# PrinceVictor/LWSNet

Measured on AMD Instinct MI355X. Metric: stereo pairs/sec @256x512 maxdisp=192 (stage-4), higher is better.
Workload: dtype f32; 1 GPU; BASELINE config 2: batch=1/GPU, 256x512 synthetic pair, maxdisplist=[24,5,5], all 4 stages; pairs_per_gpu=1, streams=1, parallelism=single GPU, weights=seeded synthetic (seed 7, calibrated BN), GPU_MAX_HW_QUEUES=4

## Files before the change

lwsnet_amd/csrc/lws_api.hip:

```cpp
#include <stdarg.h>
#include <stdio.h>
#include <string.h>

#include <algorithm>

#include "lws_common.h"

namespace lws {

static thread_local char g_err[512] = "";
thread_local hipEvent_t tl_stop_event = nullptr;

void set_error(const char *fmt, ...)
{
    va_list ap;
    va_start(ap, fmt);
    vsnprintf(g_err, sizeof(g_err), fmt, ap);
    va_end(ap);
}

static constexpr int kClockWgs = 64;

int check_device(const lws_ctx *h, const char *what)
{
    int cur = -1;
    if (hipGetDevice(&cur) != hipSuccess) {
        (void)hipGetLastError();
        cur = -1;
    }
    if (cur != h->device) {
        set_error("%s: the handle belongs to HIP device %d but the calling thread's current device is %d "
                  "(hipSetDevice(%d) first; -1 = no device)", what, h->device, cur, h->device);
        return LWS_ERR_INVALID;
    }
    return LWS_OK;
}

void apply_options(lws_ctx *h)
{
    for (int i = 0; i < 3; ++i) {
        h->stage[i].mid16_split = (h->opt.split_bf16 & 1) != 0;
        h->stage[i].mid8_split = (h->opt.split_bf16 & 2) != 0;
        h->stage[i].mid8_balance = h->mid8_balance;
        h->stage[i].cu_count = h->cu_count;
    }
    h->net2d.r2_first.form = (h->opt.split_bf16 & 4) ? 1 : 0;
}

}

using namespace lws;

extern "C" {

int lws_abi_version(void) { return LWS_ABI_VERSION; }

const char *lws_last_error(void) { return g_err; }

int lws_device_count(void)
{
    int n = 0;
    if (hipGetDeviceCount(&n) != hipSuccess) return 0;
    return n;
}

int lws_create(const lws_config *cfg, lws_handle *out)
{
    LWS_CHECK_ARG(cfg != nullptr && out != nullptr, "lws_create: null argument");
    LWS_CHECK_ARG(cfg->layers_3d >= 1 && cfg->layers_3d <= 16, "layers_3d must be in 1..16 (got %d)", cfg->layers_3d);
    LWS_CHECK_ARG(cfg->maxdisplist[0] >= 1 && cfg->maxdisplist[0] <= 64, "maxdisplist[0] must be in 1..64 (got %d)",
                  cfg->maxdisplist[0]);
    for (int i = 1; i < 3; ++i)
        LWS_CHECK_ARG(cfg->maxdisplist[i] >= 1 && 2 * cfg->maxdisplist[i] - 1 <= 64,
                      "maxdisplist[%d] must be in 1..32 (got %d)", i, cfg->maxdisplist[i]);
    for (int i = 0; i < 3; ++i) {
        const int c3 = cfg->channels_3d * cfg->growth_rate[i];
        LWS_CHECK_ARG(c3 == 8 || c3 == 16 || c3 == 32,
                      "stage %d: channels_3d*growth_rate = %d is not supported by the gfx950 kernels (8, 16, 32)", i, c3);
    }
    LWS_CHECK_ARG(cfg->feature_fp16 == 0 || cfg->feature_fp16 == 1, "feature_fp16 must be 0 or 1 (got %d)", cfg->feature_fp16);
    LWS_CHECK_ARG(cfg->interp_align_mode == 0 || cfg->interp_align_mode == 1, "interp_align_mode must be 0 or 1 (got %d)",
                  cfg->interp_align_mode);
    lws_ctx *h = new (std::nothrow) lws_ctx();
    if (!h) {
        set_error("out of host memory");
        return LWS_ERR_NOMEM;
    }
    h->cfg = *cfg;
    h->spec = build_spec(*cfg);
    for (int i = 0; i < 3; ++i) h->stage[i].c3 = cfg->channels_3d * cfg->growth_rate[i];
    if (hipGetDevice(&h->device) != hipSuccess) h->device = -1;
    (void)hipGetLastError();
    *out = h;
    return LWS_OK;
}

static int *option_slot(lws_ctx *h, const char *name)
{
    struct { const char *name; int *slot; } tab[] = {{"fuse_first", &h->opt.fuse_first},
                                                     {"defer_upsample", &h->opt.defer_upsample},
                                                     {"side_streams", &h->opt.side_streams},
                                                     {"split_bf16", &h->opt.split_bf16},
                                                     {"ref_chunk_mb", &h->opt.ref_chunk_mb},
                                                     {"ref_pipe", &h->opt.ref_pipe},
                                                     {"warp_form", &h->opt.warp_form},
                                                     {"fuse_last1", &h->opt.fuse_last1},
                                                     {"fork2_after", &h->opt.fork2_after},
                                                     {"fuse_ref_last", &h->opt.fuse_ref_last},
                                                     {"host_joins", &h->opt.host_joins},
                                                     {"host_join_budget_us", &h->opt.host_join_budget_us},
                                                     {"device", &h->device}};
    for (auto &e : tab)
        if (strcmp(e.name, name) == 0) return e.slot;
    return nullptr;
}

int lws_set_option(lws_handle h, const char *name, int value)
{
    LWS_CHECK_ARG(h && name, "lws_set_option: null argument");
    int *slot = option_slot(h, name);
    LWS_CHECK_ARG(slot != nullptr, "lws_set_option: unknown option '%s'", name);
    if (strcmp(name, "split_bf16") == 0)
        LWS_CHECK_ARG(value >= 0 && value <= 7, "lws_set_option: split_bf16 is a bit mask in 0..7 (got %d)", value);
    else if (strcmp(name, "fuse_first") == 0)
        LWS_CHECK_ARG(value >= 0 && value <= 3, "lws_set_option: fuse_first is a bit mask in 0..3 (got %d)", value);
    else if (strcmp(name, "ref_pipe") == 0 || strcmp(name, "fuse_ref_last") == 0 || strcmp(name, "host_joins") == 0)
        LWS_CHECK_ARG(value >= -1 && value <= 1, "lws_set_option: %s is out of range (got %d)", name, value);
    else if (strcmp(name, "host_join_budget_us") == 0)
        LWS_CHECK_ARG(value >= 0 && value <= 1000000, "lws_set_option: host_join_budget_us must be in 0..1000000 (got %d)", value);
    else if (strcmp(name, "ref_chunk_mb") == 0)
        LWS_CHECK_ARG(value >= 0 && value <= 4096, "lws_set_option: ref_chunk_mb must be in 0..4096 (got %d)", value);
    else if (strcmp(name, "device") == 0) {
        LWS_CHECK_ARG(value >= 0, "lws_set_option: device must be >= 0 (got %d)", value);
        LWS_CHECK_ARG(h->params == nullptr && h->ws == nullptr && h->side == nullptr,
                      "lws_set_option: the device of a handle can only be changed before lws_finalize / lws_reserve "
                      "have allocated on device %d", h->device);
    }
    else if (strcmp(name, "fork2_after") == 0)
        LWS_CHECK_ARG(value >= -1 && value <= 16, "lws_set_option: fork2_after must be in -1..16 (got %d)", value);
    else
        LWS_CHECK_ARG(value == 0 || value == 1, "lws_set_option: %s must be 0 or 1 (got %d)", name, value);
    *slot = value;
    apply_options(h);
    return LWS_OK;
}

int lws_get_option(lws_handle h, const char *name, int *value)
{
    LWS_CHECK_ARG(h && name && value, "lws_get_option: null argument");
    int *slot = option_slot(h, name);
    LWS_CHECK_ARG(slot != nullptr, "lws_get_option: unknown option '%s'", name);
    *value = *slot;
    return LWS_OK;
}

int lws_profile_enable(lws_handle h, int class_mask)
{
    LWS_CHECK_ARG(h, "lws_profile_enable: null handle");
    prof_clear(h);
    h->prof_mask = h->prof_mask_cfg = (unsigned)class_mask;
    h->prof_every = 1;
    h->prof_calls = 0;
    return LWS_OK;
}

int lws_profile_sample(lws_handle h, int every_n)
{
    LWS_CHECK_ARG(h && every_n >= 1, "lws_profile_sample: every_n must be >= 1");
    h->prof_every = every_n;
    h->prof_calls = 0;
    return LWS_OK;
}

int lws_profile_read(lws_handle h, double *total_ms, int64_t *launches)
{
    LWS_CHECK_ARG(h && total_ms && launches, "lws_profile_read: null argument");
    LWS_CHECK_DEVICE(h, "lws_profile_read");
    for (int i = 0; i < LWS_KC_COUNT; ++i) {
        total_ms[i] = 0.0;
        launches[i] = 0;
    }
    for (lws_prof_rec &r : h->prof) {
        LWS_HIP(hipEventSynchronize(r.t1));
        float ms = 0.f;
        LWS_HIP(hipEventElapsedTime(&ms, r.t0, r.t1));
        total_ms[r.kc] += ms;
        launches[r.kc] += 1;
    }
    return LWS_OK;
}

int lws_profile_read_class(lws_handle h, int kernel_class, float *ms_out, int capacity, int *count)
{
    LWS_CHECK_ARG(h && count && (ms_out || capacity == 0) && capacity >= 0, "lws_profile_read_class: bad argument");
    LWS_CHECK_ARG(kernel_class >= 0 && kernel_class < LWS_KC_COUNT, "lws_profile_read_class: unknown kernel class %d", kernel_class);
    LWS_CHECK_DEVICE(h, "lws_profile_read_class");
    int n = 0;
    for (lws_prof_rec &r : h->prof) {
        if (r.kc != kernel_class) continue;
        if (n < capacity) {
            LWS_HIP(hipEventSynchronize(r.t1));
            float ms = 0.f;
            LWS_HIP(hipEventElapsedTime(&ms, r.t0, r.t1));
            ms_out[n] = ms;
        }
        ++n;
    }
    *count = n;
    return LWS_OK;
// ... 134 lines not shown
```

lwsnet_amd/csrc/lws_common.h:

```cpp
#pragma once
#include <hip/hip_runtime.h>
#include <hip/hip_ext.h>
#include <stdint.h>

#include <atomic>
#include <map>
#include <string>
#include <type_traits>
#include <vector>

#include "lwsnet_hip.h"

namespace lws {

void set_error(const char *fmt, ...) __attribute__((format(printf, 1, 2)));

#define LWS_CHECK_ARG(cond, ...)                 \
    do {                                         \
        if (!(cond)) {                           \
            ::lws::set_error(__VA_ARGS__);       \
            return LWS_ERR_INVALID;              \
        }                                        \
    } while (0)

// ... 114 lines not shown
    }
#define LWS_STAMPK(k, i)                 \
    do {                                 \
        if ((k) == LWS_STAMPS) stamp_(i); \
    } while (0)
#else
#define LWS_DEFINE_STAMPS(tu)
#define LWS_STAMPK(k, i) do {} while (0)
#endif

struct Conv3dLayer {
    int cin = 0, cout = 0;
    float *w = nullptr;
    float *bn_s = nullptr;
    float *bn_t = nullptr;
    float *w_mfma = nullptr;
};

struct Stage3d {
    int c3 = 0;
    bool mid8_split = false;
    bool mid16_split = false;
    int mid8_balance = 1;
    int cu_count = 0;
    unsigned long long *clk = nullptr;
    std::vector<Conv3dLayer> layers;
};

struct Conv2dLayer {
    int cin = 0, cout = 0, stride = 1, pad = 1, dil = 1;
    bool transposed = false, relu = false;
    float *w = nullptr, *bn_s = nullptr, *bn_t = nullptr;
    float *w_pair = nullptr;
    float *w_mfma = nullptr;
    int pair_groups = 0;
};

struct RefDws {
    int dil = 1;
    float *bn_s = nullptr, *bn_t = nullptr;
    float *dw = nullptr;
    float *pw = nullptr;
};

struct RefConv64 {
    float *bn_s = nullptr, *bn_t = nullptr;
    float *w = nullptr;
    float *wx = nullptr;
    int form = 0;
};

struct Net2d {
    Conv2dLayer fe[12];
    float *r1_first[2] = {nullptr, nullptr};
    float *r1_first_mfma[2] = {nullptr, nullptr};
    RefDws r1[2][4];
    RefConv64 r2_first;
    RefDws r2[4];
    float *r2_last = nullptr;
};

}

struct lws_join_stat {
    int64_t host = 0, queued = 0, wait_ns = 0, max_ns = 0;
};

struct lws_prof_rec {
    int kc;
    hipEvent_t t0, t1;
};

struct lws_ctx {
    lws_config cfg;
    struct {
        int fuse_first = 3;
        int defer_upsample = 1;
        int side_streams = 1;
        int split_bf16 = 0;
        int ref_pipe = -1;
        int warp_form = 1;
        int fuse_last1 = 1;
        int fork2_after = -1;
        int fuse_ref_last = -1;
        int ref_chunk_mb = 72;
        int host_joins = -1;
        int host_join_budget_us = 900;
    } opt;
    lws_join_stat join_stat[3];
    unsigned prof_mask = 0;
    unsigned prof_mask_cfg = 0;
    int prof_every = 1;
    unsigned prof_calls = 0;
    std::vector<lws_prof_rec> prof;
    std::vector<hipEvent_t> evt_pool;
    int device = 0;
    int cu_count = 0;
    bool finalized = false;
    std::map<std::string, std::vector<float>> host;
    std::map<std::string, std::vector<int64_t>> shapes;
    std::map<std::string, std::vector<int64_t>> spec;
    float *params = nullptr;
    bool owns_params = true;
    size_t params_bytes = 0;
    lws::Stage3d stage[3];
    lws::Net2d net2d;
    bool have_2d = false;
    float *ws = nullptr;
    size_t ws_bytes = 0;
    int mid8_balance = 1;
    hipStream_t side = nullptr;
    hipEvent_t ev_fork = nullptr, ev_join = nullptr;
    hipEvent_t ev_feat[3] = {nullptr, nullptr, nullptr};
    hipEvent_t ev_fork2 = nullptr;
    unsigned long long *clk_buf = nullptr;
};

namespace lws {

struct StageMap {
    float *mem = nullptr;
    bool written = false;
    const float *low = nullptr;
    int h = 0, w = 0;
    StageMap *prev = nullptr;
};
int check_stage_map(const StageMap &m, bool nested, const char *who);

int check_device(const lws_ctx *h, const char *what);
#define LWS_CHECK_DEVICE(h, what)                     \
    do {                                              \
        int rc_dev_ = ::lws::check_device((h), what); \
        if (rc_dev_) return rc_dev_;                  \
    } while (0)
void apply_options(lws_ctx *h);
void prof_clear(lws_ctx *h);
std::map<std::string, std::vector<int64_t>> build_spec(const lws_config &cfg);

int launch_volume_l1_shift(const float *L, const float *R, float *cost, int B, int C, int h, int w, int D,
                           hipStream_t st, bool q16 = false);
int launch_volume_l1_warp(const float *L, const float *R, StageMap &prev, float *cost, float *wflow_out,
                          int B, int C, int h, int w, int H, int W, int m, hipStream_t st, bool q16 = false,
                          int form = 1,
                          float ioff = 0.5f);
int launch_softargmin(const float *cost, float *low, int B, int D, int h, int w, float start, hipStream_t st);
int launch_upsample_add(const float *low, const float *prev, float *out, int B, int h, int w, int H, int W,
                        hipStream_t st, float ioff = 0.5f);
int launch_softargmin_upsample(const float *cost, const float *prev, float *out, float *low_out, int B, int D, int h,
                               int w, int H, int W, float start, hipStream_t st, float ioff = 0.5f);
int launch_softargmin_conf(const float *cost, float *disp_low, float *peak_low, float *sigma_low, float *conf, float *sigma, int B,
                           int D, int h, int w, int H, int W, float start, hipStream_t st, float ioff = 0.5f);

bool shift_first_can_fuse(const Stage3d &s, int C);
int launch_shift_first(const Stage3d &s, const float *L, const float *R, float *cost, float *act_out, int B, int C, int D,
                       int h, int w, hipStream_t st, bool q16);
int launch_conv3d_first(const Stage3d &s, const float *cost, float *act_out, int B, int D, int h, int w,
                        hipStream_t st);
int launch_conv3d_mid(const Stage3d &s, int layer, const float *act_in, float *act_out, int B, int D, int h,
                      int w, hipStream_t st, hipEvent_t e0 = nullptr, hipEvent_t e1 = nullptr);
int launch_conv3d_last(const Stage3d &s, const float *act_in, const float *cost_skip, float *cost_out, int B,
                       int D, int h, int w, hipStream_t st);

int launch_conv2d_nchw(const Conv2dLayer &l, const float *in, const float *res, float *out, int N, int H, int W,
                       hipStream_t st, const float *in2 = nullptr, int n1 = 0);
int conv2d_pair_groups(int layer);
void pack_pair_mfma(const float *w, int cin, float *out);
// ... 30 lines not shown
```

lwsnet_amd/csrc/lws_feature2d.hip:

```cpp
#include "lws_common.h"
#include "lws_device_math.h"

namespace lws {

LWS_DEFINE_STAMPS(feature2d)

template <int CIN, int COUT, bool TRANSPOSED>
__global__ __launch_bounds__(256) void k_conv2d_nchw(const float *__restrict__ in, const float *__restrict__ in2, int n1,
                                                     const float *__restrict__ wgt,
                                                     const float *__restrict__ bn_s, const float *__restrict__ bn_t,
                                                     const float *__restrict__ res, float *__restrict__ out, int H,
                                                     int W, int Ho, int Wo, int stride, int pad, int dil, int relu,
                                                     int RH, int RW, int RWp)
{
    constexpr int CPT = COUT / 4;
    extern __shared__ float sIn[];
    const int b = blockIdx.z;
    const int tid = threadIdx.x, tx = tid & 7, ty = (tid >> 3) & 7;
    const int wave_id = __builtin_amdgcn_readfirstlane(tid >> 6);
    const int co0 = wave_id * CPT;
    const int ox0 = blockIdx.x * 8, oy0 = blockIdx.y * 8;
    const int ry0 = TRANSPOSED ? ((oy0 - 1) >> 1) : oy0 * stride - pad;
    const int rx0 = TRANSPOSED ? ((ox0 - 1) >> 1) : ox0 * stride - pad;
    const int plane = H * W, oplane = Ho * Wo;
    const float *inb = b < n1 ? in + (int64_t)b * CIN * plane : in2 + (int64_t)(b - n1) * CIN * plane;
    LWS_STAMPK(7, 0);
    const int rsz = RH * RW;
#pragma unroll
    for (int k = 0; k < 2; ++k) {
        const int r = tid + 256 * k;
        if (r < rsz) {
            const int ry = r / RW, rx = r - ry * RW;
            const int gy = ry0 + ry, gx = rx0 + rx;
            const bool ok = gy >= 0 && gy < H && gx >= 0 && gx < W;
            const float *src = inb + (ok ? gy * W + gx : 0);
            float v[CIN];
#pragma unroll
            for (int ci = 0; ci < CIN; ++ci) v[ci] = src[ci * plane];
            float *dst = sIn + ry * RWp + rx;
#pragma unroll
            for (int ci = 0; ci < CIN; ++ci) dst[ci * RH * RWp] = ok ? v[ci] : 0.0f;
        }
    }
    __syncthreads();
    LWS_STAMPK(7, 1);
    const int ox = ox0 + tx, oy = oy0 + ty;
    if (ox >= Wo || oy >= Ho) return;
    float acc[CPT];
#pragma unroll
    for (int c = 0; c < CPT; ++c) acc[c] = 0.0f;
    const int cstride = RH * RWp;
#pragma unroll 3
    for (int tap = 0; tap < 9; ++tap) {
        const int kh = tap / 3, kw = tap - kh * 3;
        int ly, lx;
        bool ok = true;
        if (TRANSPOSED) {
            const int t_y = oy + 1 - kh, t_x = ox + 1 - kw;
            ok = t_y >= 0 && !(t_y & 1) && (t_y >> 1) < H && t_x >= 0 && !(t_x & 1) && (t_x >> 1) < W;
            ly = (t_y >> 1) - ry0;
            lx = (t_x >> 1) - rx0;
        } else {
            ly = ty * stride + kh * dil;
            lx = tx * stride + kw * dil;
        }
        const float *p = sIn + (ok ? ly * RWp + lx : 0);
        const float *w = wgt + (tap * 4 + wave_id) * CIN * CPT;
        float v[CIN];
#pragma unroll
        for (int ci = 0; ci < CIN; ++ci) v[ci] = ok ? p[ci * cstride] : 0.0f;
#pragma unroll
        for (int ci = 0; ci < CIN; ++ci)
#pragma unroll
            for (int c = 0; c < CPT; ++c) acc[c] = fmaf(v[ci], w[ci * CPT + c], acc[c]);
    }
    LWS_STAMPK(7, 2);
    const int64_t o = ((int64_t)b * COUT + co0) * oplane + oy * Wo + ox;
#pragma unroll
    for (int c = 0; c < CPT; ++c) {
        float v = acc[c];
        if (bn_s != nullptr) v = fmaf(v, bn_s[co0 + c], bn_t[co0 + c]);
        if (res != nullptr) v = v + res[o + (int64_t)c * oplane];
        if (relu) v = fmaxf(v, 0.0f);
        out[o + (int64_t)c * oplane] = v;
    }
    LWS_STAMPK(7, 3);
}

template <int CIN, int COUT, bool TR>
static int conv2d_launch(const Conv2dLayer &l, const float *in, const float *in2, int n1, const float *res, float *out,
                         int N, int H, int W, int Ho, int Wo, hipStream_t st)
{
    const int RH = TR ? 6 : 7 * l.stride + 2 * l.dil + 1, RW = RH;
    const int RWp = RW | 1;
    const size_t lds = (size_t)CIN * RH * RWp * sizeof(float);
    dim3 grid(cdiv(Wo, 8), cdiv(Ho, 8), N), block(256);
    hipLaunchKernelGGL((k_conv2d_nchw<CIN, COUT, TR>), grid, block, lds, st, in, in2, n1, l.w, l.bn_s, l.bn_t, res, out, H,
                       W, Ho, Wo, l.stride, l.pad, l.dil, l.relu ? 1 : 0, RH, RW, RWp);
    LWS_LAUNCH_CHECK();
    return LWS_OK;
}

int launch_conv2d_nchw(const Conv2dLayer &l, const float *in, const float *res, float *out, int N, int H, int W,
                       hipStream_t st, const float *in2, int n1)
{
    if (in2 == nullptr) {
        in2 = in;
        n1 = N;
    }
    int Ho, Wo;
    if (l.transposed) {
        Ho = 2 * H;
        Wo = 2 * W;
    } else {
        Ho = (H + 2 * l.pad - 2 * l.dil - 1) / l.stride + 1;
        Wo = (W + 2 * l.pad - 2 * l.dil - 1) / l.stride + 1;
    }
#define LWS_C2D(CI, CO, TR)                                   \
    if (l.cin == CI && l.cout == CO && l.transposed == TR)    \
        return conv2d_launch<CI, CO, TR>(l, in, in2, n1, res, out, N, H, W, Ho, Wo, st);
    LWS_C2D(3, 4, false) LWS_C2D(4, 8, false) LWS_C2D(8, 4, false) LWS_C2D(8, 16, false) LWS_C2D(16, 16, false)
    LWS_C2D(16, 16, true) LWS_C2D(16, 8, true) LWS_C2D(8, 8, false)
#undef LWS_C2D
    set_error("conv2d_nchw: unsupported layer cin=%d cout=%d", l.cin, l.cout);
    return LWS_ERR_INVALID;
}

template <int CIN, int CM, int COUT, int SA, int DA, int DB, int NW>
struct PairCfg {
    static constexpr int NT = 64 * NW;
    static constexpr int MR = 8 + 2 * DB, MRp = MR | 1;
    static constexpr int RH = (MR - 1) * SA + 2 * DA + 1;
    static constexpr int HALF = (RH + 1) / 2, RWp = (SA == 2 ? 2 * HALF : RH) | 1;
    __host__ __device__ static constexpr int col(int rx) { return SA == 2 ? (rx & 1) * HALF + (rx >> 1) : rx; }
    static constexpr int WGA_ = (MR * MR + 63) / 64;
    static constexpr int WGA = WGA_ <= 1 ? 1 : WGA_ <= 2 ? 2 : WGA_ <= 4 ? 4 : WGA_ <= 8 ? 8 : 16;
    static constexpr int GA = NW / WGA, CPA = CM / GA, CPB = COUT / NW;
    static constexpr int ITEMS = CIN * RH * RH, SITER = (ITEMS + NT - 1) / NT;
    static constexpr int LDS_FLOATS = CIN * RH * RWp + CM * MR * MRp;
    static_assert(WGA <= NW && NW % WGA == 0 && CM % GA == 0 && COUT % NW == 0 && CPA >= 1 && CPB >= 1, "bad pair geometry");
    static_assert(WGA * 64 >= MR * MR, "phase 2 must be one pass");
};

template <int CIN, int CM, int COUT, int SA, int DA, int DB, int NW>
__global__ __launch_bounds__(64 * NW) void k_conv2d_pair(const float *__restrict__ in, const float *__restrict__ in2, int n1,
                                                         const float *__restrict__ wA, const float *__restrict__ sA_,
                                                         const float *__restrict__ tA_, int reluA,
                                                         const float *__restrict__ wB, const float *__restrict__ sB_,
                                                         const float *__restrict__ tB_, const float *__restrict__ res,
                                                         int reluB, float *__restrict__ out, int H, int W, int HA, int WA)
{
    using Cfg = PairCfg<CIN, CM, COUT, SA, DA, DB, NW>;
    constexpr int NT = Cfg::NT, MR = Cfg::MR, MRp = Cfg::MRp, RH = Cfg::RH, RWp = Cfg::RWp, WGA = Cfg::WGA, GA = Cfg::GA,
                  CPA = Cfg::CPA, CPB = Cfg::CPB, SITER = Cfg::SITER, RSZ = RH * RH;
    extern __shared__ float smem[];
    float *sIn = smem;
    float *sMid = smem + CIN * RH * RWp;
    const int b = blockIdx.z;
    const int tid = threadIdx.x, lane = tid & 63, wave = __builtin_amdgcn_readfirstlane(tid >> 6);
    const int ox0 = blockIdx.x * 8, oy0 = blockIdx.y * 8;
    const int my0 = oy0 - DB, mx0 = ox0 - DB;
    const int iy0 = my0 * SA - DA, ix0 = mx0 * SA - DA;
    const int plane = H * W;
    const float *inb = b < n1 ? in + (int64_t)b * CIN * plane : in2 + (int64_t)(b - n1) * CIN * plane;
    [[maybe_unused]] constexpr int STAMP_ID = 13 + (CIN == 3 ? 0 : CM == 4 ? 1 : CIN == 8 ? 2 : 3);
    LWS_STAMPK(STAMP_ID, 0);
    {
        float v[SITER];
        bool okv[SITER];
#pragma unroll
        for (int i = 0; i < SITER; ++i) {
            const int it = tid + i * NT;
            const int ci = it / RSZ, r = it - ci * RSZ;
            const int ry = r / RH, rx = r - ry * RH;
            const int gy = iy0 + ry, gx = ix0 + rx;
            okv[i] = it < Cfg::ITEMS && gy >= 0 && gy < H && gx >= 0 && gx < W;
            v[i] = inb[okv[i] ? ci * plane + gy * W + gx : 0];
        }
#pragma unroll
        for (int i = 0; i < SITER; ++i) {
            const int it = tid + i * NT;
            const int ci = it / RSZ, r = it - ci * RSZ;
            const int ry = r / RH, rx = r - ry * RH;
            if (it < Cfg::ITEMS) sIn[(ci * RH + ry) * RWp + Cfg::col(rx)] = okv[i] ? v[i] : 0.0f;
        }
    }
    __syncthreads();
    LWS_STAMPK(STAMP_ID, 1);
    {
        const int ga = wave / WGA;
        const int coA = ga * CPA;
        const int p = (wave - ga * WGA) * 64 + lane;
        if (p < MR * MR) {
            const int my = p / MR, mx = p - my * MR;
            const int ay = my0 + my, ax = mx0 + mx;
            const bool valid = ay >= 0 && ay < HA && ax >= 0 && ax < WA;
            float acc[CPA];
#pragma unroll
            for (int c = 0; c < CPA; ++c) acc[c] = 0.0f;
#pragma unroll 3
            for (int tap = 0; tap < 9; ++tap) {
                const int kh = tap / 3, kw = tap - kh * 3;
                const float *pp = sIn + (my * SA + kh * DA) * RWp + Cfg::col(mx * SA + kw * DA);
                const float *w = wA + (tap * GA + ga) * CIN * CPA;
                float v[CIN];
// ... 267 lines not shown
```

lwsnet_amd/csrc/lws_forward.hip:

```cpp
#include <algorithm>
#include <chrono>

#include "lws_common.h"

namespace lws {

struct WsLayout {
    size_t act_a, act_b, cost_raw, cost_out, low[3], total;
    size_t fe_o, fe_o2, fe_pre, fe_f8, fe_f4, fe_o3, fe_cls, fe_f2;
    size_t r_a, r_b, r_c;
    size_t total_all;
};

static inline int half_up(int v) { return (v + 1) / 2; }

static inline float ioff_of(const lws_ctx *h) { return h->cfg.interp_align_mode == 1 ? 0.0f : 0.5f; }

struct StageDims {
    int D, hh, ww;
    float start;
};
static StageDims stage_dims(const lws_ctx *h, int s, int H, int W)
{
    const int div = 4 >> s, m = h->cfg.maxdisplist[s];
// ... 472 lines not shown
    if (rc) return rc;
    const WsLayout L = ws_layout(h, B, H, W);
    rc = begin_call(h, "lws_disparity_stages", false, "disparity_stages: lws_finalize has not been called", L.total);
    if (rc) return rc;
    hipStream_t st = (hipStream_t)stream;
    StageMap map[3] = {{pred_out[0]}, {pred_out[1]}, {pred_out[2]}};
    for (int s = 0; s < 3; ++s) {
        const bool defer = defers(h, s, B, H, W, s == 1);
        const StageDims d = stage_dims(h, s, H, W);
        bool fused;
        rc = stage_volume(h, s, d, featsL[s], featsR[s], B, H, W, map, L, st, defer, fused);
        if (rc) return rc;
        rc = stage_map(h, s, d, B, H, W, map, L, st, defer, fused);
        if (rc) return rc;
    }
    return LWS_OK;
}

int lws_feature_extraction(lws_handle h, const float *img, int N, int H, int W, float *f8, float *f4, float *f2,
                           void *stream)
{
    LWS_CHECK_ARG(h && img && f8 && f4 && f2, "feature_extraction: null pointer");
    LWS_CHECK_ARG(N >= 1 && size_ok(H, W),
                  "feature_extraction: unsupported size N=%d %dx%d (ceil(H/2), ceil(W/2) divisible by 4)", N, H, W);
    const WsLayout L = ws_layout(h, (N + 1) / 2, H, W);
    int rc = begin_call(h, "lws_feature_extraction", true,
                        "feature_extraction: the 2D network tensors were not all set before lws_finalize", L.total_all);
    if (rc) return rc;
    hipStream_t st = (hipStream_t)stream;
    rc = feature_head(h, img, nullptr, N, 0, H, W, L, f8, st);
    if (rc) return rc;
    return feature_tail(h, N, H, W, L, f8, f4, f2, st, nullptr, 3);
}

int lws_refine(lws_handle h, const float *left, const float *pred3, int B, int H, int W, float *pred4, void *stream)
{
    LWS_CHECK_ARG(h && left && pred3 && pred4, "refine: null pointer");
    LWS_CHECK_ARG(B >= 1 && H > 0 && W > 0, "refine: unsupported size B=%d %dx%d", B, H, W);
    const WsLayout L = ws_layout(h, B, H, W);
    int rc = begin_call(h, "lws_refine", true, "refine: the 2D network tensors were not all set before lws_finalize",
                        L.total_all);
    if (rc) return rc;
    rc = refine_left(h, left, B, H, W, L, (hipStream_t)stream);
    if (rc) return rc;
    const StageMap p3{const_cast<float *>(pred3), true};
    return refine_rest(h, p3, B, H, W, L, pred4, (hipStream_t)stream);
}

}

struct ConfOut {
    float *const *conf;
    float *const *sigma;
};

static int run_forward(lws_ctx *h, const char *what, const float *left, const float *right, int B, int H, int W,
                       float *const pred_out[4], const ConfOut *co, hipStream_t st)
{
    const WsLayout L = ws_layout(h, B, H, W);
    int rc = begin_call(h, what, true, "forward: set_state_dict/lws_finalize must be called with the full state dict first",
                        L.total_all);
    if (rc) return rc;
    bool capturing = false;
    if (st != nullptr) {
        hipStreamCaptureStatus cs = hipStreamCaptureStatusNone;
        LWS_HIP(hipStreamIsCapturing(st, &cs));
        capturing = cs != hipStreamCaptureStatusNone;
    }
    struct MaskGuard {
        lws_ctx *h;
        ~MaskGuard() { h->prof_mask = h->prof_mask_cfg; }
    } mask_guard{h};
    h->prof_mask = (!capturing && (h->prof_every <= 1 || h->prof_calls++ % (unsigned)h->prof_every == 0)) ? h->prof_mask_cfg : 0u;
    const bool multi = h->opt.side_streams != 0;
    if (multi) {
        rc = ensure_streams(h);
        if (rc) return rc;
    }
    hipStream_t side = multi ? h->side : st;
    const bool ext = multi && !capturing;
    const bool same_handle = tl_last_forward == h;
    tl_last_forward = h;
    bool hj = !capturing && (h->opt.host_joins >= 0 ? h->opt.host_joins != 0 : B == 1 && same_handle);
    float *f8 = h->ws + L.fe_f8, *f4 = h->ws + L.fe_f4, *f2 = h->ws + L.fe_f2;
    rc = feature_head(h, left, right, B, B, H, W, L, f8, st, Fork{multi ? h->ev_feat[0] : nullptr, 0, ext});
    if (rc) return rc;
    const size_t n2 = (size_t)B * 8 * half_up(H) * half_up(W), n4 = n2 / 2, n8 = n2 / 8;
    const float *fl[3] = {f8, f4, f2};
    const float *fr[3] = {f8 + n8, f4 + n4, f2 + n2};
    if (multi) LWS_HIP(hipStreamWaitEvent(side, h->ev_feat[0], 0));
    rc = feature_tail(h, 2 * B, H, W, L, f8, f4, f2, side, multi ? h->ev_feat : nullptr, 1);
    if (rc) return rc;
    const int L3 = h->cfg.layers_3d;
    int fork2 = h->opt.fork2_after;
    if (fork2 < 0) fork2 = L3;
    if (fork2 > L3) fork2 = 0;
    const bool ref_evaluates = (h->opt.fuse_first & 1) && ref_first_dws_can_fuse(h->net2d.r1[1][0], 1);
    StageMap map[3] = {{pred_out[0]}, {pred_out[1]}, {pred_out[2]}};
    for (int s = 0; s < 3; ++s) {
        if (multi && s > 0) {
            rc = host_join(h, s - 1, h->ev_feat[s], st, hj);
            if (rc) return rc;
        }
        const bool defer = co == nullptr && defers(h, s, B, H, W, s < 2 || ref_evaluates);
        const StageDims d = stage_dims(h, s, H, W);
        bool fused;
        rc = stage_volume(h, s, d, fl[s], fr[s], B, H, W, map, L, st, defer, fused,
                          Fork{multi && s == 0 ? h->ev_fork2 : nullptr, fork2, ext}, co != nullptr);
        if (rc) return rc;
        if (s == 0) {
            if (multi) LWS_HIP(hipStreamWaitEvent(side, h->ev_fork2, 0));
            rc = feature_tail(h, 2 * B, H, W, L, f8, f4, f2, side, multi ? h->ev_feat : nullptr, 2);
            if (rc) return rc;
            rc = refine_left(h, left, B, H, W, L, side);
            if (rc) return rc;
            if (multi) LWS_HIP(hipEventRecord(h->ev_join, side));
        }
        rc = stage_map(h, s, d, B, H, W, map, L, st, defer, fused);
        if (rc) return rc;
        float *conf = co != nullptr && co->conf != nullptr ? co->conf[s] : nullptr;
        float *sigma = co != nullptr && co->sigma != nullptr ? co->sigma[s] : nullptr;
        if (conf != nullptr || sigma != nullptr) {
            ProfScope p(h, LWS_KC_CONFIDENCE, st);
            rc = launch_softargmin_conf(h->ws + L.cost_out, nullptr, nullptr, nullptr, conf, sigma, B, d.D, d.hh, d.ww, H, W,
                                        d.start, st, ioff_of(h));
            if (rc) return rc;
        }
    }
    if (multi) {
        rc = host_join(h, 2, h->ev_join, st, hj);
        if (rc) return rc;
    }
    return refine_rest(h, map[2], B, H, W, L, pred_out[3], st);
}

extern "C" {

int lws_forward(lws_handle h, const float *left, const float *right, int B, int H, int W, float *const pred_out[4],
                void *stream)
{
    LWS_CHECK_ARG(h && left && right && pred_out, "forward: null pointer");
    for (int s = 0; s < 4; ++s) LWS_CHECK_ARG(pred_out[s], "forward: null output for stage %d", s + 1);
    const int rc = check_size(h, B, H, W);
    if (rc) return rc;
    return run_forward(h, "lws_forward", left, right, B, H, W, pred_out, nullptr, (hipStream_t)stream);
}

int lws_forward_conf(lws_handle h, const float *left, const float *right, int B, int H, int W, float *const pred_out[4],
                     float *const conf_out[3], float *const sigma_out[3], void *stream)
{
    LWS_CHECK_ARG(h && left && right && pred_out, "forward_conf: null pointer");
    for (int s = 0; s < 4; ++s) LWS_CHECK_ARG(pred_out[s], "forward_conf: null output for stage %d", s + 1);
    LWS_CHECK_ARG(B <= 65535, "forward_conf: batch %d above 65535", B);
    const int rc = check_size(h, B, H, W);
    if (rc) return rc;
    const ConfOut co{conf_out, sigma_out};
    return run_forward(h, "lws_forward_conf", left, right, B, H, W, pred_out, &co, (hipStream_t)stream);
}

}
```

lwsnet_amd/csrc/lws_params.hip:

```cpp
#include <math.h>
#include <string.h>

#include "lws_common.h"

namespace lws {

typedef std::map<std::string, std::vector<int64_t>> Spec;

static void spec_bn(Spec &sp, const std::string &p, int c)
{
    for (const char *s : {".weight", ".bias", "._mean", "._variance"}) sp[p + s] = {c};
}

static const struct { const char *name; int cin, cout, stride, pad, dil; bool tr, bn, relu; } kFeLayers[12] = {
    {"dres0.0", 3, 4, 2, 2, 2, false, true, true},         {"dres0.2", 4, 8, 1, 4, 4, false, true, true},
    {"dres1.0", 8, 4, 1, 2, 2, false, true, true},         {"dres1.2", 4, 8, 1, 2, 2, false, true, false},
    {"dres2.conv1.0", 8, 16, 2, 1, 1, false, true, true},  {"dres2.conv2.0", 16, 16, 1, 1, 1, false, true, true},
    {"dres2.conv3.0", 16, 16, 2, 1, 1, false, true, true}, {"dres2.conv4.0", 16, 16, 1, 1, 1, false, true, true},
    {"dres2.conv5", 16, 16, 2, 1, 1, true, true, true},    {"dres2.conv6", 16, 8, 2, 1, 1, true, true, false},
    {"classif1.0", 8, 8, 1, 1, 1, false, true, true},      {"classif1.2", 8, 8, 1, 1, 1, false, false, false}};

static std::string fe_name(int i) { return std::string("feature_extraction.") + kFeLayers[i].name; }
static std::string fe_weight_key(int i) { return fe_name(i) + (kFeLayers[i].bn ? ".0.weight" : ".weight"); }

// ... 59 lines not shown
    void align() { slab.resize((slab.size() + 63) & ~(size_t)63, 0.0f); }
    void put(const std::vector<float> &v, float *&dst)
    {
        align();
        refs.push_back({&dst, slab.size()});
        slab.insert(slab.end(), v.begin(), v.end());
    }
    void put_bn(const lws_ctx *h, const std::string &p, float *&s_dst, float *&t_dst)
    {
        std::vector<float> s, t;
        fold_bn(h, p, s, t);
        put(s, s_dst);
        put(t, t_dst);
    }
    void bind(float *base)
    {
        for (const auto &r : refs) *r.first = base + r.second;
    }
};

static void pack_net3d(lws_ctx *h, SlabBuilder &sb)
{
    const int L = h->cfg.layers_3d + 2;
    for (int i = 0; i < 3; ++i) {
        const int c3 = h->stage[i].c3;
        h->stage[i].layers.assign(L, Conv3dLayer());
        for (int j = 0; j < L; ++j) {
            Conv3dLayer &l = h->stage[i].layers[j];
            l.cin = j == 0 ? 1 : c3;
            l.cout = j == L - 1 ? 1 : c3;
            const std::vector<float> &w = h->host.at(vp_name(i, j) + ".2.weight");
            if (j == 0) {
                sb.put(w, l.w);
                std::vector<float> wf(c3 == 8 ? 9 * 64 : (size_t)(c3 / 16) * 7 * 64);
                if (c3 == 8)
                    pack_first8_weights(w.data(), wf.data());
                else
                    pack_first16_weights(w.data(), c3, wf.data());
                sb.put(wf, l.w_mfma);
            } else if (j == L - 1) {
                std::vector<float> wt((size_t)27 * c3);
                for (int ci = 0; ci < c3; ++ci)
                    for (int tap = 0; tap < 27; ++tap) wt[(size_t)tap * c3 + ci] = w[(size_t)ci * 27 + tap];
                sb.put(wt, l.w);
            } else {
                std::vector<float> wp(packed_mid_weight_floats(c3));
                pack_mid_weights(w.data(), c3, wp.data());
                sb.put(wp, l.w);
            }
            sb.put_bn(h, vp_name(i, j) + ".0", l.bn_s, l.bn_t);
        }
    }
}

static void pack_dws(const lws_ctx *h, SlabBuilder &sb, const DwsKeys &k, int dil, RefDws &r)
{
    r.dil = dil;
    sb.put_bn(h, k.bn, r.bn_s, r.bn_t);
    const std::vector<float> &dw = h->host.at(k.dw);
    std::vector<float> dwt(9 * 32);
    for (int c = 0; c < 32; ++c)
        for (int tap = 0; tap < 9; ++tap) dwt[tap * 32 + c] = dw[c * 9 + tap];
    sb.put(dwt, r.dw);
    std::vector<float> pw(2 * 2 * 64 * 4);
    pack_conv2d_mfma(h->host.at(k.pw).data(), 32, 1, pw.data());
    sb.put(pw, r.pw);
}

static void pack_net2d(lws_ctx *h, SlabBuilder &sb)
{
    Net2d &n = h->net2d;
    n = Net2d();
    for (int i = 0; i < 12; ++i) {
        const auto &d = kFeLayers[i];
        Conv2dLayer &l = n.fe[i];
        l.cin = d.cin; l.cout = d.cout; l.stride = d.stride; l.pad = d.pad; l.dil = d.dil;
        l.transposed = d.tr; l.relu = d.relu;
        const std::vector<float> &w = h->host.at(fe_weight_key(i));
        const int cpt = d.cout / 4;
        std::vector<float> wt((size_t)9 * d.cin * d.cout);
        for (int co = 0; co < d.cout; ++co)
            for (int ci = 0; ci < d.cin; ++ci)
                for (int tap = 0; tap < 9; ++tap)
                    wt[(((size_t)tap * 4 + co / cpt) * d.cin + ci) * cpt + co % cpt] =
                        d.tr ? w[((size_t)ci * d.cout + co) * 9 + tap] : w[((size_t)co * d.cin + ci) * 9 + tap];
        sb.put(wt, l.w);
        const int G = l.pair_groups = conv2d_pair_groups(i);
        if (G > 0) {
            const int cpg = d.cout / G;
            std::vector<float> wq((size_t)9 * d.cin * d.cout);
            for (int co = 0; co < d.cout; ++co)
                for (int ci = 0; ci < d.cin; ++ci)
                    for (int tap = 0; tap < 9; ++tap)
                        wq[(((size_t)tap * G + co / cpg) * d.cin + ci) * cpg + co % cpg] = w[((size_t)co * d.cin + ci) * 9 + tap];
            sb.put(wq, l.w_pair);
        }
        if (i >= 4 && i <= 7) {
            std::vector<float> wf((size_t)9 * 64 * (d.cin / 4));
            pack_pair_mfma(w.data(), d.cin, wf.data());
            sb.put(wf, l.w_mfma);
        }
        if (d.bn) sb.put_bn(h, fe_name(i) + ".1", l.bn_s, l.bn_t);
    }
    for (int k = 0; k < 2; ++k) {
        const int cin = k == 0 ? 3 : 1;
        const std::vector<float> &w = h->host.at(std::string(kRef1[k]) + ".0.weight");
        std::vector<float> wt(9 * cin * 32);
        for (int co = 0; co < 32; ++co)
            for (int ci = 0; ci < cin; ++ci)
                for (int tap = 0; tap < 9; ++tap) wt[(tap * cin + ci) * 32 + co] = w[(co * cin + ci) * 9 + tap];
        sb.put(wt, n.r1_first[k]);
        std::vector<float> wf(packed_first_mfma_floats(cin));
        pack_first_mfma(w.data(), cin, wf.data());
        sb.put(wf, n.r1_first_mfma[k]);
        for (int b = 0; b < 4; ++b) pack_dws(h, sb, dws_keys(kRef1[k], b + 1), 2 << b, n.r1[k][b]);
    }
    {
        sb.put_bn(h, "refinement2.0.0", n.r2_first.bn_s, n.r2_first.bn_t);
        const std::vector<float> &w = h->host.at("refinement2.0.2.weight");
        std::vector<float> wp(10 * 4 * 2 * 64 * 4, 0.0f);
        pack_conv2d_mfma(w.data(), 64, 9, wp.data());
        sb.put(wp, n.r2_first.w);
        std::vector<float> wx(packed_conv64x_floats(), 0.0f);
        pack_conv64_bf16x3(w.data(), wx.data());
        sb.put(wx, n.r2_first.wx);
    }
    for (int b = 0; b < 4; ++b) pack_dws(h, sb, dws_keys("refinement2", b + 1), 8 >> b, n.r2[b]);
    {
        const std::vector<float> &w = h->host.at("refinement2.5.weight");
        std::vector<float> wt(9 * 32);
        for (int ci = 0; ci < 32; ++ci)
            for (int tap = 0; tap < 9; ++tap) wt[tap * 32 + ci] = w[ci * 9 + tap];
        sb.put(wt, n.r2_last);
    }
}

}

using namespace lws;

extern "C" {

int lws_set_tensor(lws_handle h, const char *key, const float *host, const int64_t *shape, int ndim)
{
    LWS_CHECK_ARG(h && key && host && shape && ndim >= 1 && ndim <= 5, "lws_set_tensor: bad argument");
    if (!h->owns_params) {
        set_error("lws_set_tensor: this handle is a clone and shares its source's parameters");
        return LWS_ERR_STATE;
    }
    auto it = h->spec.find(key);
    LWS_CHECK_ARG(it != h->spec.end(), "set_state_dict: unexpected key '%s'", key);
    std::vector<int64_t> shp(shape, shape + ndim);
    if (shp != it->second) {
        std::string want, got;
        for (int64_t d : it->second) want += std::to_string(d) + ",";
        for (int64_t d : shp) got += std::to_string(d) + ",";
        set_error("set_state_dict: shape mismatch for '%s': expected [%s] got [%s]", key, want.c_str(), got.c_str());
        return LWS_ERR_INVALID;
    }
    size_t n = 1;
    for (int64_t d : shp) n *= (size_t)d;
    h->host[key].assign(host, host + n);
    h->shapes[key] = shp;
    h->finalized = false;
    return LWS_OK;
}

int lws_finalize(lws_handle h)
// ... 41 lines not shown
```

Measured before the change: 2201 pairs/s.

## Add dedicated stride-2 deconv kernel and rework feature-tail fork scheduling

Replaces the generic transposed-convolution path, which evaluated all 9 taps per output with parity masking, with a dedicated stride-2 deconvolution kernel. Each thread computes one input pixel's 2x2 output quad using only the taps that contribute, and weights are repacked per tap/cout/cin. It also adds a fork1 option that can defer the feature tail to the later fork, and sets fork2 to default to 0 when batch is 1. These change the stream overlap schedule as well as cutting wasted deconvolution arithmetic, at some risk of worse overlap on the side stream.

```diff
diff --git a/lwsnet_amd/csrc/lws_api.hip b/lwsnet_amd/csrc/lws_api.hip
--- a/lwsnet_amd/csrc/lws_api.hip
+++ b/lwsnet_amd/csrc/lws_api.hip
@@ -106,6 +106,7 @@
                                                      {"warp_form", &h->opt.warp_form},
                                                      {"fuse_last1", &h->opt.fuse_last1},
                                                      {"fork2_after", &h->opt.fork2_after},
+                                                     {"fork1", &h->opt.fork1},
                                                      {"fuse_ref_last", &h->opt.fuse_ref_last},
                                                      {"host_joins", &h->opt.host_joins},
                                                      {"host_join_budget_us", &h->opt.host_join_budget_us},
@@ -124,7 +125,8 @@
         LWS_CHECK_ARG(value >= 0 && value <= 7, "lws_set_option: split_bf16 is a bit mask in 0..7 (got %d)", value);
     else if (strcmp(name, "fuse_first") == 0)
         LWS_CHECK_ARG(value >= 0 && value <= 3, "lws_set_option: fuse_first is a bit mask in 0..3 (got %d)", value);
-    else if (strcmp(name, "ref_pipe") == 0 || strcmp(name, "fuse_ref_last") == 0 || strcmp(name, "host_joins") == 0)
+    else if (strcmp(name, "ref_pipe") == 0 || strcmp(name, "fuse_ref_last") == 0 || strcmp(name, "host_joins") == 0 ||
+             strcmp(name, "fork1") == 0)
         LWS_CHECK_ARG(value >= -1 && value <= 1, "lws_set_option: %s is out of range (got %d)", name, value);
     else if (strcmp(name, "host_join_budget_us") == 0)
         LWS_CHECK_ARG(value >= 0 && value <= 1000000, "lws_set_option: host_join_budget_us must be in 0..1000000 (got %d)", value);
diff --git a/lwsnet_amd/csrc/lws_common.h b/lwsnet_amd/csrc/lws_common.h
--- a/lwsnet_amd/csrc/lws_common.h
+++ b/lwsnet_amd/csrc/lws_common.h
@@ -220,6 +220,7 @@
         int warp_form = 1;
         int fuse_last1 = 1;
         int fork2_after = -1;
+        int fork1 = -1;
         int fuse_ref_last = -1;
         int ref_chunk_mb = 72;
         int host_joins = -1;
diff --git a/lwsnet_amd/csrc/lws_feature2d.hip b/lwsnet_amd/csrc/lws_feature2d.hip
--- a/lwsnet_amd/csrc/lws_feature2d.hip
+++ b/lwsnet_amd/csrc/lws_feature2d.hip
@@ -5,7 +5,7 @@
 
 LWS_DEFINE_STAMPS(feature2d)
 
-template <int CIN, int COUT, bool TRANSPOSED>
+template <int CIN, int COUT>
 __global__ __launch_bounds__(256) void k_conv2d_nchw(const float *__restrict__ in, const float *__restrict__ in2, int n1,
                                                      const float *__restrict__ wgt,
                                                      const float *__restrict__ bn_s, const float *__restrict__ bn_t,
@@ -20,8 +20,8 @@
     const int wave_id = __builtin_amdgcn_readfirstlane(tid >> 6);
     const int co0 = wave_id * CPT;
     const int ox0 = blockIdx.x * 8, oy0 = blockIdx.y * 8;
-    const int ry0 = TRANSPOSED ? ((oy0 - 1) >> 1) : oy0 * stride - pad;
-    const int rx0 = TRANSPOSED ? ((ox0 - 1) >> 1) : ox0 * stride - pad;
+    const int ry0 = oy0 * stride - pad;
+    const int rx0 = ox0 * stride - pad;
     const int plane = H * W, oplane = Ho * Wo;
     const float *inb = b < n1 ? in + (int64_t)b * CIN * plane : in2 + (int64_t)(b - n1) * CIN * plane;
     LWS_STAMPK(7, 0);
@@ -53,22 +53,11 @@
 #pragma unroll 3
     for (int tap = 0; tap < 9; ++tap) {
         const int kh = tap / 3, kw = tap - kh * 3;
-        int ly, lx;
-        bool ok = true;
-        if (TRANSPOSED) {
-            const int t_y = oy + 1 - kh, t_x = ox + 1 - kw;
-            ok = t_y >= 0 && !(t_y & 1) && (t_y >> 1) < H && t_x >= 0 && !(t_x & 1) && (t_x >> 1) < W;
-            ly = (t_y >> 1) - ry0;
-            lx = (t_x >> 1) - rx0;
-        } else {
-            ly = ty * stride + kh * dil;
-            lx = tx * stride + kw * dil;
-        }
-        const float *p = sIn + (ok ? ly * RWp + lx : 0);
+        const float *p = sIn + (ty * stride + kh * dil) * RWp + tx * stride + kw * dil;
         const float *w = wgt + (tap * 4 + wave_id) * CIN * CPT;
         float v[CIN];
 #pragma unroll
-        for (int ci = 0; ci < CIN; ++ci) v[ci] = ok ? p[ci * cstride] : 0.0f;
+        for (int ci = 0; ci < CIN; ++ci) v[ci] = p[ci * cstride];
 #pragma unroll
         for (int ci = 0; ci < CIN; ++ci)
 #pragma unroll
@@ -87,16 +76,116 @@
     LWS_STAMPK(7, 3);
 }
 
-template <int CIN, int COUT, bool TR>
+template <int CIN, int COUT>
 static int conv2d_launch(const Conv2dLayer &l, const float *in, const float *in2, int n1, const float *res, float *out,
                          int N, int H, int W, int Ho, int Wo, hipStream_t st)
 {
-    const int RH = TR ? 6 : 7 * l.stride + 2 * l.dil + 1, RW = RH;
+    const int RH = 7 * l.stride + 2 * l.dil + 1, RW = RH;
     const int RWp = RW | 1;
     const size_t lds = (size_t)CIN * RH * RWp * sizeof(float);
     dim3 grid(cdiv(Wo, 8), cdiv(Ho, 8), N), block(256);
-    hipLaunchKernelGGL((k_conv2d_nchw<CIN, COUT, TR>), grid, block, lds, st, in, in2, n1, l.w, l.bn_s, l.bn_t, res, out, H,
+    hipLaunchKernelGGL((k_conv2d_nchw<CIN, COUT>), grid, block, lds, st, in, in2, n1, l.w, l.bn_s, l.bn_t, res, out, H,
                        W, Ho, Wo, l.stride, l.pad, l.dil, l.relu ? 1 : 0, RH, RW, RWp);
+    LWS_LAUNCH_CHECK();
+    return LWS_OK;
+}
+
+template <int CIN, int COUT>
+struct DeconvCfg {
+    static constexpr int NW = 4, NT = 64 * NW, GROUPS = COUT / NW;
+    static constexpr int RH = 9, RWp = 24;
+    static constexpr int PL = RH * RWp, ITEMS = CIN * RH * RH, SITER = (ITEMS + NT - 1) / NT;
+    static_assert(COUT % NW == 0, "bad deconvolution geometry");
+};
+
+template <int CIN, int COUT>
+__global__ __launch_bounds__(256) void k_deconv2d_s2(const float *__restrict__ in, const float *__restrict__ wgt,
+                                                     const float *__restrict__ bn_s, const float *__restrict__ bn_t,
+                                                     const float *__restrict__ res, float *__restrict__ out, int H, int W,
+                                                     int relu)
+{
+    using Cfg = DeconvCfg<CIN, COUT>;
+    constexpr int NT = Cfg::NT, RH = Cfg::RH, RWp = Cfg::RWp, PL = Cfg::PL, SITER = Cfg::SITER;
+    __shared__ float sIn[CIN * PL];
+    const int b = blockIdx.z / Cfg::GROUPS, grp = blockIdx.z - b * Cfg::GROUPS;
+    const int tid = threadIdx.x, lane = tid & 63;
+    const int co = grp * Cfg::NW + __builtin_amdgcn_readfirstlane(tid >> 6);
+    const int cx0 = blockIdx.x * 8, cy0 = blockIdx.y * 8;
+    const int Wo = 2 * W, plane = H * W;
+    const int64_t oplane = (int64_t)4 * plane;
+    const float *inb = in + (int64_t)b * CIN * plane;
+    float v[SITER];
+    bool okv[SITER];
+#pragma unroll
+    for (int i = 0; i < SITER; ++i) {
+        const int it = tid + i * NT;
+        const int ci = it / (RH * RH), r = it - ci * (RH * RH);
+        const int ry = r / RH, rx = r - ry * RH;
+        const int gy = cy0 + ry, gx = cx0 + rx;
+        okv[i] = it < Cfg::ITEMS && gy < H && gx < W;
+        v[i] = inb[okv[i] ? ci * plane + gy * W + gx : 0];
+    }
+    const int cy = lane >> 3, cx = lane & 7;
+    const int iy = cy0 + cy, ix = cx0 + cx;
+    const bool live = iy < H && ix < W;
+    const int64_t o = ((int64_t)b * COUT + co) * oplane + (int64_t)(2 * iy) * Wo + 2 * ix;
+    float rv[4];
+#pragma unroll
+    for (int q = 0; q < 4; ++q) rv[q] = (res != nullptr && live) ? res[o + (q >> 1) * Wo + (q & 1)] : 0.0f;
+#pragma unroll
+    for (int i = 0; i < SITER; ++i) {
+        const int it = tid + i * NT;
+        const int ci = it / (RH * RH), r = it - ci * (RH * RH);
+        const int ry = r / RH, rx = r - ry * RH;
+        if (it < Cfg::ITEMS) sIn[ci * PL + ry * RWp + rx] = okv[i] ? v[i] : 0.0f;
+    }
+    __syncthreads();
+    if (!live) return;
+    float x[2][2][CIN];
+    const float *p = sIn + cy * RWp + cx;
+#pragma unroll
+    for (int ci = 0; ci < CIN; ++ci) {
+        x[0][0][ci] = p[ci * PL];
+        x[0][1][ci] = p[ci * PL + 1];
+        x[1][0][ci] = p[ci * PL + RWp];
+        x[1][1][ci] = p[ci * PL + RWp + 1];
+    }
+    const float s = bn_s != nullptr ? bn_s[co] : 1.0f, t = bn_s != nullptr ? bn_t[co] : 0.0f;
+#pragma unroll
+    for (int q = 0; q < 4; ++q) {
+        const int py = q >> 1, px = q & 1;
+        float acc = 0.0f;
+#pragma unroll
+        for (int kh = 0; kh < 3; ++kh) {
+            if ((kh == 1) != (py == 0)) continue;
+#pragma unroll
+            for (int kw = 0; kw < 3; ++kw) {
+                if ((kw == 1) != (px == 0)) continue;
+                const float *xs = x[kh == 0 ? 1 : 0][kw == 0 ? 1 : 0];
+                const float *w = wgt + ((kh * 3 + kw) * COUT + co) * CIN;
+#pragma unroll
+                for (int ci = 0; ci < CIN; ++ci) acc = fmaf(xs[ci], w[ci], acc);
+            }
+        }
+        float r = acc;
+        if (bn_s != nullptr) r = fmaf(r, s, t);
+        if (res != nullptr) r = r + rv[q];
+        if (relu) r = fmaxf(r, 0.0f);
+        out[o + py * Wo + px] = r;
+    }
+}
+
+template <int CIN, int COUT>
+static int deconv2d_launch(const Conv2dLayer &l, const float *in, const float *res, float *out, int N, int H, int W,
+                           hipStream_t st)
+{
+    using Cfg = DeconvCfg<CIN, COUT>;
+    if ((int64_t)N * Cfg::GROUPS > 65535) {
+        set_error("conv2d_nchw: %d images are too many for one transposed-convolution launch", N);
+        return LWS_ERR_INVALID;
+    }
+    dim3 grid(cdiv(W, 8), cdiv(H, 8), N * Cfg::GROUPS), block(Cfg::NT);
+    hipLaunchKernelGGL((k_deconv2d_s2<CIN, COUT>), grid, block, 0, st, in, l.w, l.bn_s, l.bn_t, res, out, H, W, l.relu ? 1 : 0);
     LWS_LAUNCH_CHECK();
     return LWS_OK;
 }
@@ -116,11 +205,18 @@
         Ho = (H + 2 * l.pad - 2 * l.dil - 1) / l.stride + 1;
         Wo = (W + 2 * l.pad - 2 * l.dil - 1) / l.stride + 1;
     }
-#define LWS_C2D(CI, CO, TR)                                   \
-    if (l.cin == CI && l.cout == CO && l.transposed == TR)    \
-        return conv2d_launch<CI, CO, TR>(l, in, in2, n1, res, out, N, H, W, Ho, Wo, st);
-    LWS_C2D(3, 4, false) LWS_C2D(4, 8, false) LWS_C2D(8, 4, false) LWS_C2D(8, 16, false) LWS_C2D(16, 16, false)
-    LWS_C2D(16, 16, true) LWS_C2D(16, 8, true) LWS_C2D(8, 8, false)
+    if (l.transposed) {
+        if (in2 != in) {
+            set_error("conv2d_nchw: a transposed layer reads one input tensor");
+            return LWS_ERR_INVALID;
+        }
+        if (l.cin == 16 && l.cout == 16) return deconv2d_launch<16, 16>(l, in, res, out, N, H, W, st);
+        if (l.cin == 16 && l.cout == 8) return deconv2d_launch<16, 8>(l, in, res, out, N, H, W, st);
+    }
+#define LWS_C2D(CI, CO)                                        \
+    if (l.cin == CI && l.cout == CO && !l.transposed)          \
+        return conv2d_launch<CI, CO>(l, in, in2, n1, res, out, N, H, W, Ho, Wo, st);
+    LWS_C2D(3, 4) LWS_C2D(4, 8) LWS_C2D(8, 4) LWS_C2D(8, 16) LWS_C2D(16, 16) LWS_C2D(8, 8)
 #undef LWS_C2D
     set_error("conv2d_nchw: unsupported layer cin=%d cout=%d", l.cin, l.cout);
     return LWS_ERR_INVALID;
diff --git a/lwsnet_amd/csrc/lws_forward.hip b/lwsnet_amd/csrc/lws_forward.hip
--- a/lwsnet_amd/csrc/lws_forward.hip
+++ b/lwsnet_amd/csrc/lws_forward.hip
@@ -578,18 +578,21 @@
     const bool same_handle = tl_last_forward == h;
     tl_last_forward = h;
     bool hj = !capturing && (h->opt.host_joins >= 0 ? h->opt.host_joins != 0 : B == 1 && same_handle);
+    const int L3 = h->cfg.layers_3d;
+    const bool fork1 = !multi || h->opt.fork1 != 0;
     float *f8 = h->ws + L.fe_f8, *f4 = h->ws + L.fe_f4, *f2 = h->ws + L.fe_f2;
-    rc = feature_head(h, left, right, B, B, H, W, L, f8, st, Fork{multi ? h->ev_feat[0] : nullptr, 0, ext});
+    rc = feature_head(h, left, right, B, B, H, W, L, f8, st, Fork{multi && fork1 ? h->ev_feat[0] : nullptr, 0, ext});
     if (rc) return rc;
     const size_t n2 = (size_t)B * 8 * half_up(H) * half_up(W), n4 = n2 / 2, n8 = n2 / 8;
     const float *fl[3] = {f8, f4, f2};
     const float *fr[3] = {f8 + n8, f4 + n4, f2 + n2};
-    if (multi) LWS_HIP(hipStreamWaitEvent(side, h->ev_feat[0], 0));
-    rc = feature_tail(h, 2 * B, H, W, L, f8, f4, f2, side, multi ? h->ev_feat : nullptr, 1);
-    if (rc) return rc;
-    const int L3 = h->cfg.layers_3d;
+    if (fork1) {
+        if (multi) LWS_HIP(hipStreamWaitEvent(side, h->ev_feat[0], 0));
+        rc = feature_tail(h, 2 * B, H, W, L, f8, f4, f2, side, multi ? h->ev_feat : nullptr, 1);
+        if (rc) return rc;
+    }
     int fork2 = h->opt.fork2_after;
-    if (fork2 < 0) fork2 = L3;
+    if (fork2 < 0) fork2 = B == 1 ? 0 : L3;
     if (fork2 > L3) fork2 = 0;
     const bool ref_evaluates = (h->opt.fuse_first & 1) && ref_first_dws_can_fuse(h->net2d.r1[1][0], 1);
     StageMap map[3] = {{pred_out[0]}, {pred_out[1]}, {pred_out[2]}};
@@ -606,7 +609,7 @@
         if (rc) return rc;
         if (s == 0) {
             if (multi) LWS_HIP(hipStreamWaitEvent(side, h->ev_fork2, 0));
-            rc = feature_tail(h, 2 * B, H, W, L, f8, f4, f2, side, multi ? h->ev_feat : nullptr, 2);
+            rc = feature_tail(h, 2 * B, H, W, L, f8, f4, f2, side, multi ? h->ev_feat : nullptr, fork1 ? 2 : 3);
             if (rc) return rc;
             rc = refine_left(h, left, B, H, W, L, side);
             if (rc) return rc;
diff --git a/lwsnet_amd/csrc/lws_params.hip b/lwsnet_amd/csrc/lws_params.hip
--- a/lwsnet_amd/csrc/lws_params.hip
+++ b/lwsnet_amd/csrc/lws_params.hip
@@ -165,8 +165,10 @@
         for (int co = 0; co < d.cout; ++co)
             for (int ci = 0; ci < d.cin; ++ci)
                 for (int tap = 0; tap < 9; ++tap)
-                    wt[(((size_t)tap * 4 + co / cpt) * d.cin + ci) * cpt + co % cpt] =
-                        d.tr ? w[((size_t)ci * d.cout + co) * 9 + tap] : w[((size_t)co * d.cin + ci) * 9 + tap];
+                    if (d.tr)
+                        wt[((size_t)tap * d.cout + co) * d.cin + ci] = w[((size_t)ci * d.cout + co) * 9 + tap];
+                    else
+                        wt[(((size_t)tap * 4 + co / cpt) * d.cin + ci) * cpt + co % cpt] = w[((size_t)co * d.cin + ci) * 9 + tap];
         sb.put(wt, l.w);
         const int G = l.pair_groups = conv2d_pair_groups(i);
         if (G > 0) {
```

After: 2198 pairs/s. No clear change (-0.1%).
